# prsinha1/Distributed-Inverse-Problem-Admm

Hardware: AMD Instinct MI355X
Metric: ADMM node-updates/sec (whole node), 512² phantom; rel-Fro vs CPU ref (higher is better)
Workload: dtype f32 samples / f64 state; 1 GPU; C3 (BASELINE.json configs[2] 512^2, 16 graph nodes (ring), 96 angles/node, float32 samples, iso TV, lam=0.02 rho=2, split-Bregman 10x5 CG) on 1 GPU(s), one step = one outer ADMM iteration; image=512, nodes=16, angles_per_node=96, graph=ring, parallelism=graph-node shards x1, batch_streams=1

## Files before the change

### distributed-inverse-problem-admm_amd/admm_hip/_lib.py

```python
from __future__ import annotations

import ctypes as C
import os
import threading

_HERE = os.path.dirname(os.path.abspath(__file__))
LIB_NAME = "libadmm_tomo.so"
LIB_PATH = os.path.join(_HERE, LIB_NAME)

ADMM_DTYPE_F32 = 0
ADMM_DTYPE_F64 = 1
ADMM_TV_ISO = 0
ADMM_TV_ANISO = 1
ADMM_FUSE_MIDPOINT = 0
ADMM_FUSE_WEIGHTED = 1
ADMM_BATCH_KEEP_X = 1
ABI_VERSION = 9
ADMM_MASK_KNN = 0
ADMM_MASK_MST = 1
ADMM_MASK_CHAIN = 2
ADMM_Q_ARITHMETIC = 0
ADMM_Q_HARMONIC = 1
MASK_MAX_NODES = 64
ADMM_FBP_RAMLAK = 0
# ... 52 lines not shown
        ("inc_off", C.c_void_p),
        ("inc_edge", C.c_void_p),
        ("inc_qslot", C.c_void_p),
        ("inc_sign", C.c_void_p),
        ("node_stats", C.c_void_p),
        ("edge_stats", C.c_void_p),
        ("fusion", C.c_int32),
        ("flags", C.c_int32),
        ("y_b", C.c_void_p),
        ("w", C.c_void_p),
        ("x_prev", C.c_void_p),
    ]


SYMBOLS = {
    "admm_abi_version": [],
    "admm_last_error": [],
    "admm_ctx_create": [C.POINTER(C.c_void_p), C.POINTER(Geom), C.c_int, C.c_int, C.c_int],
    "admm_ctx_create_matrix": [C.POINTER(C.c_void_p), C.c_int, C.c_int, C.c_longlong, C.c_void_p, C.c_void_p,
                               C.c_void_p, C.c_int, C.c_int, C.c_int],
    "admm_ctx_destroy": [C.c_void_p],
    "admm_project_fwd": [C.c_void_p, C.c_void_p, C.c_void_p, C.c_int, C.c_void_p],
    "admm_project_adj": [C.c_void_p, C.c_void_p, C.c_void_p, C.c_int, C.c_void_p],
    "admm_column_norms_sq": [C.c_void_p, C.c_void_p, C.c_void_p],
    "admm_tv_grad": [C.c_void_p, C.c_void_p, C.c_void_p, C.c_void_p, C.c_int, C.c_void_p],
    "admm_tv_div": [C.c_void_p, C.c_void_p, C.c_void_p, C.c_void_p, C.c_int, C.c_void_p],
    "admm_batch_bind": [C.c_void_p, C.POINTER(Batch)],
    "admm_batch_atb": [C.c_void_p, C.c_void_p, C.c_void_p],
    "admm_node_update": [C.c_void_p, C.c_void_p],
    "admm_node_update_rounds": [C.c_void_p, C.c_int, C.c_void_p],
    "admm_consensus": [C.c_void_p, C.c_void_p],
    "admm_time_forward": [C.c_void_p, C.c_int, C.c_int, C.c_void_p, C.POINTER(C.c_double)],
    "admm_batch_info": [C.c_void_p, C.POINTER(C.c_int), C.POINTER(C.c_int)],
    "admm_time_back": [C.c_void_p, C.c_void_p, C.POINTER(C.c_double)],
    "admm_consensus_range": [C.c_void_p, C.c_int, C.c_int, C.c_int, C.c_void_p],
    "admm_fwd_plan_info": [C.c_void_p, C.c_int, C.POINTER(C.c_int), C.POINTER(C.c_int),
                           C.POINTER(C.c_double), C.POINTER(C.c_int)],
    "admm_pixel_masks": [C.c_void_p, C.c_int, C.c_int64, C.c_int, C.c_int, C.c_int, C.c_void_p,
                         C.c_void_p, C.c_void_p],
    "admm_chain_orders": [C.POINTER(C.c_uint64), C.c_int, C.c_uint32, C.c_int, C.c_int64, C.c_void_p,
                          C.POINTER(C.c_uint64)],
    "admm_fbp_filter": [C.c_void_p, C.c_void_p, C.c_int, C.c_int, C.c_int, C.c_int, C.c_double, C.c_double,
                        C.c_int, C.c_void_p],
    "admm_image_metrics": [C.c_void_p, C.c_longlong, C.c_void_p, C.c_void_p, C.c_int, C.c_int, C.c_double,
                           C.c_double, C.c_void_p, C.c_void_p, C.c_void_p],
    "admm_image_metrics_work": [C.c_int, C.c_int, C.POINTER(C.c_longlong)],
    "admm_batch_set_ray_weights": [C.c_void_p, C.c_void_p, C.c_void_p],
    "admm_column_norms_sq_weighted": [C.c_void_p, C.c_void_p, C.c_void_p, C.c_void_p],
    "admm_bound_project": [C.c_void_p, C.c_longlong, C.c_void_p, C.c_void_p, C.c_longlong, C.c_void_p, C.c_void_p,
                           C.c_double, C.c_double, C.c_longlong, C.c_int, C.c_void_p, C.c_void_p, C.c_void_p],
    "admm_bound_project_work": [C.c_longlong, C.c_int, C.POINTER(C.c_longlong)],
    "admm_consensus_relaxed": [C.c_void_p, C.c_longlong, C.c_int, C.c_void_p, C.c_void_p, C.c_void_p, C.c_void_p,
                               C.c_void_p, C.c_void_p, C.c_int, C.c_int, C.c_double, C.c_void_p, C.c_void_p,
                               C.c_void_p],
    "admm_consensus_relaxed_work": [C.c_longlong, C.c_int, C.POINTER(C.c_longlong)],
    "admm_bound_project_relaxed": [C.c_void_p, C.c_longlong, C.c_void_p, C.c_void_p, C.c_longlong, C.c_void_p,
                                   C.c_void_p, C.c_double, C.c_double, C.c_longlong, C.c_int, C.c_double, C.c_void_p,
                                   C.c_void_p, C.c_void_p],
    "admm_batch_set_rho": [C.c_void_p, C.c_double, C.c_void_p],
    "admm_node_norms": [C.c_void_p, C.c_longlong, C.c_void_p, C.c_void_p, C.c_void_p, C.c_longlong, C.c_int,
                        C.c_void_p, C.c_void_p, C.c_void_p, C.c_int, C.c_void_p, C.c_void_p, C.c_void_p],
    "admm_node_norms_work": [C.c_longlong, C.c_int, C.POINTER(C.c_longlong)],
    "admm_fuse_absmax": [C.c_void_p, C.c_longlong, C.c_void_p, C.c_longlong, C.c_void_p, C.c_longlong, C.c_int,
                         C.c_int, C.c_void_p, C.c_void_p, C.c_void_p],
    "admm_fuse_absmax_work": [C.c_longlong, C.c_int, C.POINTER(C.c_longlong)],
    "admm_fuse_accumulate": [C.c_void_p, C.c_longlong, C.c_void_p, C.c_longlong, C.c_void_p, C.c_longlong, C.c_int,
# ... 62 lines not shown
```

### distributed-inverse-problem-admm_amd/csrc/admm_tomo.hip

```cpp
#include <hip/hip_runtime.h>

#include <algorithm>
#include <cmath>
#include <cstdio>
#include <cstdlib>
#include <cstring>
#include <initializer_list>
#include <memory>
#include <string>
#include <type_traits>
#include <utility>
#include <vector>

#include "../../include/admm_tomo.h"
#include "fwd_plan.hpp"
#include "kernels.hpp"

using namespace admm;

static_assert(sizeof(FgBlock) == sizeof(int4) && alignof(FgBlock) == alignof(int4), "FgBlock must be an int4");

namespace {
thread_local std::string g_err;

// ... 146 lines not shown
  int wexp = 0;
  static constexpr int kPlans = kFwdPlans;
  FwdPlan plans[kPlans];
  Buf plan_groups_b[kPlans], plan_rng_b[kPlans];
  const FgGroup* plan_groups(int pl) const { return plan_groups_b[pl].as<const FgGroup>(); }
  const FgRange* plan_rng(int pl) const { return plan_rng_b[pl].as<const FgRange>(); }
  int plan_n[kPlans] = {}, plan_blocks[kPlans] = {};
  double plan_staged[kPlans] = {};
  const FgGroup* groups = nullptr;
  const FgRange* rng = nullptr;
  int n_groups = 0;
  bool mirror_half = false;
  Buf fg_order;
  int fg_nblk = 0, fg_order_nch = 0;
  int fg_cpb = 1;
  Stream cap;

  bool csr = false;
  long long nnz = 0;
  Buf f_ptr, f_idx, f_val, t_ptr, t_idx, t_val;

  Buf op_img, op_imgT, op_sino, op_fpart;
  Buf op_order[kPlans];
  int op_nblk[kPlans] = {};
  int op_fpart_key = -1;

  bool bound = false;
  admm_batch b{};
  int vb = 1;
  bool mm = false;
  int bk_staging = 0;
  bool bk_epi_lds = true;
  int n_cu = 0;
  std::unique_ptr<admm_ctx> half;
  Buf xs, xsT, p, pT, Hp, sino, bI, fpart, r, c, d2, e2;
  Buf dsumS;
  Buf wS;
  bool weighted = false;
  Buf x2, p2;
  Buf pring;
  Buf ats;
  std::vector<Event>* tf_ev = nullptr;
  size_t tf_next = 0;
  int tf_kind = 0;
  bool ats_valid = false;
  bool ats_stale = false;
  Buf partH, partS, partD, partE;
  Buf redH;
  int P_back = 0, P_tile = 0, P_fwd = 0, P_edge = 0;
  Graph upd, upd_reuse, cons;

  admm_ctx() = default;
  admm_ctx(const admm_ctx&) = delete;
  admm_ctx& operator=(const admm_ctx&) = delete;
  ~admm_ctx() {
    scope.enter(device);
    (void)hipDeviceSynchronize();
    half.reset();
  }
};

namespace {

int vb_for(int V, int dtype) {
  const int vb = V >= 5 ? 8 : (V >= 3 ? 4 : (V == 2 ? 2 : 1));
  return dtype == ADMM_DTYPE_F64 ? std::min(vb, 4) : vb;
// ... 281 lines not shown
        }
      }
      hipLaunchKernelGGL(kern, grid, dim3(kBkThreads), 0, s, a);
      CHECK_LAUNCH();
      return ADMM_OK;
    }
  }
  back_geom(a, C, C, V);
  const int N = C->g.N;
  constexpr bool kOneImage = MODE == BACK_WSQ || MODE == BACK_WSQW;
  dim3 grid((N + kBTJ - 1) / kBTJ, (N + kBTI - 1) / kBTI, kOneImage ? 1 : (V + VB - 1) / VB);
  if (C->csr) {
    a.csr_ptr = (const int*)C->t_ptr.p;
    a.csr_idx = (const int*)C->t_idx.p;
    a.csr_val = (const T*)C->t_val.p;
    hipLaunchKernelGGL((k_back<T, VB, MODE, true>), grid, dim3(kBkThreads), 0, s, a);
  } else {
    hipLaunchKernelGGL((k_back<T, VB, MODE>), grid, dim3(kBkThreads), 0, s, a);
  }
  CHECK_LAUNCH();
  return ADMM_OK;
}

int back_partitions(admm_ctx* C) {
  const int N = C->g.N;
  const int rows = C->mm ? (N + 1) / 2 : N;
  return ((N + kBTJ - 1) / kBTJ) * ((rows + kBTI - 1) / kBTI);
}
dim3 tile_grid(admm_ctx* C, int nchunks, int vb) {
  const int N = C->g.N, ti = kTile / vb;
  return dim3((N + kTile - 1) / kTile, (N + ti - 1) / ti, nchunks);
}

int launch_reduce(const double* part, int rows, int P, double* out, int G, int ostride, int ooff, hipStream_t s) {
  hipLaunchKernelGGL(k_reduce_rows, dim3(rows), dim3(kBlock), 0, s, part, P, out, G, ostride, ooff);
  CHECK_LAUNCH();
  return ADMM_OK;
}

EdgeIn edge_in(const admm_batch& B) {
  EdgeIn E{};
  E.z = B.z;
  E.y = B.y;
  E.yb = B.fusion == ADMM_FUSE_WEIGHTED ? B.y_b : nullptr;
  E.xp = B.x_prev;
  E.ea = B.edge_a;
  E.eb = B.edge_b;
  return E;
}

template <typename T, int VB>
auto tv_kernel(bool last, bool uin, bool uout) {
  if (last) return uin ? k_tv_update<T, VB, true, true, false> : k_tv_update<T, VB, true, false, false>;
  if (uin) return k_tv_update<T, VB, false, true, true>;
  return uout ? k_tv_update<T, VB, false, false, true> : k_tv_update<T, VB, false, false, false>;
}

template <typename T, int VB>
int enqueue_update(admm_ctx* C, hipStream_t s, bool reuse = false, int rounds = 0) {
  const admm_batch& B = C->b;
  const int V = B.V, N = C->g.N;
  const size_t npix = (size_t)N * N;
  const int nch = (V + VB - 1) / VB;
  T* xs = (T*)C->xs.p;
  T* xsT = (T*)C->xsT.p;
  T* p = (T*)C->p.p;
  T* pT = (T*)C->pT.p;
  T* Hp = (T*)C->Hp.p;
  T* sino = (T*)C->sino.p;
  double* r = (double*)C->r.p;
  double* c = (double*)C->c.p;
  double* redH = (double*)C->redH.p;
  const dim3 tg = tile_grid(C, nch, VB);
  const dim3 cgg((N + kTile - 1) / kTile, (N + kCgRows - 1) / kCgRows, nch);
  const dim3 tvg((N + kTvTile - 1) / kTvTile, (N + EwMap<VB>::TI - 1) / EwMap<VB>::TI, nch);
  const int Pb = C->P_back;

  if (reuse) {
    hipLaunchKernelGGL((k_start_reuse<T, VB>), cgg, dim3(kBlock), 0, s, (const T*)C->ats.p, B.x_ext, edge_in(B),
                       B.q, B.inc_off, B.inc_edge, B.inc_qslot, B.inc_sign, B.atb, c, B.dsum, B.d, B.e, r, p, pT,
                       B.rho, B.mu, N, V);
    CHECK_LAUNCH();
  } else {
  hipLaunchKernelGGL((k_gather<T, VB>), tg, dim3(kBlock), 0, s, B.x_ext, edge_in(B), B.q, B.inc_off, B.inc_edge,
                     B.inc_qslot, B.inc_sign, c, xs, xsT, N, V);
  CHECK_LAUNCH();
  RET((launch_fwd_batch<T, VB, 0>(C, xs, xsT, sino, nullptr, nullptr, V, s)));
  {
    BackArgs<T> a{};
    a.sino = sino;
    a.out_t = p;
    a.out_d = r;
    a.pin = xs;
    a.dsum = B.dsum;
    a.atb = B.atb;
    a.cvec = c;
    a.dvar = B.d;
    a.evar = B.e;
    a.rho = B.rho;
    a.lam = B.lam;
    a.mu = B.mu;
    RET((launch_back<T, VB, BACK_INIT>(C, a, V, s)));
  }
  hipLaunchKernelGGL((k_transpose<T, VB>), tg, dim3(kBlock), 0, s, p, pT, N);
  CHECK_LAUNCH();
  }

  const double tau = B.lam / B.mu;
// ... 27 lines not shown
      a.dsum_s = (const T*)C->dsumS.p;
      a.rho = B.rho;
      a.lam = B.lam;
      a.mu = B.mu;
      Event* bev = nullptr;
      if (C->tf_ev && C->tf_kind == 1 && C->tf_next + 2 <= C->tf_ev->size()) {
        bev = C->tf_ev->data() + C->tf_next;
        C->tf_next += 2;
        HIPCHK(hipEventRecord(bev[0].e, s));
      }
      RET((launch_back<T, VB, BACK_H>(C, a, V, s)));
      if (bev) HIPCHK(hipEventRecord(bev[1].e, s));
      RET(launch_reduce((double*)C->partH.p, 5 * V, Pb, rk, 1, 1, 0, s));
      if (kk + 1 < K) {
        const auto cg = (F == 2) ? k_cg_update<T, VB, false> : k_cg_update<T, VB, true>;
        hipLaunchKernelGGL(cg, cgg, dim3(kBlock), 0, s, xcur, r, pk, pT, Hp, rk, N, V, (F == 2) ? slot[kk + 1] : pk);
        CHECK_LAUNCH();
      }
    }
    const bool last = (t + 1 == Tt);
    PRing<T> pr{};
    pr.K = (F == 2) ? K : 1;
    for (int k = 0; k < pr.K; ++k) pr.p[k] = slot[k];
    T* pout = last ? xs : (F == 2 ? slot[K] : (F == 1 ? slot[1] : slot[0]));
    T* poutT = last ? xsT : pT;
    const bool uin = t > 0 && Tt > 1;
    const bool uout = !last && Tt > 1;
    double* ua = (double*)C->d2.p;
    double* ub = (double*)C->e2.p;
    const double* din = uin ? ((t % 2) ? ua : ub) : dcur;
    const double* ein = ecur;
    double* dout = uout ? ((t % 2) ? ub : ua) : (Tt > 1 ? B.d : dnxt);
    double* eout = uout ? nullptr : (Tt > 1 ? B.e : enxt);
    hipLaunchKernelGGL((tv_kernel<T, VB>(last, uin, uout)), tvg, dim3(kTvThreads), 0, s, xcur, din, ein, dout, eout, r,
                       pout, poutT, tau, B.mu, B.tv_kind, N, V, xnxt, pr, Hp, redH);
    CHECK_LAUNCH();
    if (Tt == 1) {
      std::swap(dcur, dnxt);
      std::swap(ecur, enxt);
    }
    std::swap(xcur, xnxt);
    if (!last) std::swap(slot[0], slot[F == 2 ? K : 1]);
  }
  if (xcur != B.x_ext)
    HIPCHK(hipMemcpyAsync(B.x_ext, xcur, (size_t)V * npix * sizeof(double), hipMemcpyDeviceToDevice, s));
  if (dcur != B.d) {
    HIPCHK(hipMemcpyAsync(B.d, dcur, 2 * V * npix * sizeof(double), hipMemcpyDeviceToDevice, s));
    HIPCHK(hipMemcpyAsync(B.e, ecur, 2 * V * npix * sizeof(double), hipMemcpyDeviceToDevice, s));
  }
  RET((launch_fwd_batch<T, VB, 1>(C, xs, xsT, sino, (const T*)B.b, (double*)C->partS.p, V, s)));
  {
    BackArgs<T> a{};
    a.sino = sino;
    a.part = (double*)C->partD.p;
    a.dsum = B.dsum;
    a.cvec = c;
    a.x = B.x_ext;
    a.phantom = B.phantom;
    a.edges = edge_in(B);
    a.qv = B.q;
    a.inc_off = B.inc_off;
    a.inc_edge = B.inc_edge;
    a.inc_qslot = B.inc_qslot;
    a.inc_sign = B.inc_sign;
    a.rho = B.rho;
    a.lam = B.lam;
    a.mu = B.mu;
    a.tv_kind = B.tv_kind;
// ... 142 lines not shown
  RET(ensure(C->op_sino, vbmax * m * ds));
  RET(ensure(C->op_fpart, (size_t)kFgSeg * vbmax * m * ds));
  for (int v0 = 0; v0 < nimg; v0 += step) {
    const int nc = std::min(step, nimg - v0);
    const T* in = img + (size_t)v0 * npix;
    T* out = sino + (size_t)v0 * m;
    RET(with_vb(vb_for(nc, C->dtype), [&](auto vbc) { return op_forward_chunk<T, decltype(vbc)::value>(C, in, out, nc, s); }));
  }
  return ADMM_OK;
}

}

extern "C" {

int admm_abi_version(void) { return ADMM_ABI_VERSION; }
const char* admm_last_error(void) { return g_err.c_str(); }

int admm_ctx_create(admm_ctx** out, const admm_geom* geom, int dtype, int max_images, int device) {
  if (!out || !geom) return fail(ADMM_E_INVALID, "null argument");
  *out = nullptr;
  const admm_geom g = *geom;
  if (const char* err = check_geom(g, dtype, max_images)) return fail(ADMM_E_INVALID, err);
  GeomTables T;
  if (const char* err = geom_tables(g, dtype, T)) return fail(ADMM_E_INVALID, err);
  FwdPlans P = build_fwd_plans(g, T.fa);
  DEVICE_SCOPE(device);
  std::unique_ptr<admm_ctx> C(new admm_ctx());
  C->g = g;
  C->dtype = dtype;
  C->device = device;
  C->bk_staging = env_word("ADMM_BK_STAGING", {"reg", "dma1", "dma2"});
  C->bk_epi_lds = env_word("ADMM_BK_EPI", {"global"}) == 0;
  HIPCHK(hipDeviceGetAttribute(&C->n_cu, hipDeviceAttributeMultiprocessorCount, device));
  C->max_images = max_images;
  C->npix = g.N * g.N;
  C->mrays = g.n_angles * g.n_det;
  C->Kb = T.Kb;
  C->kbias = T.kbias;
  C->wexp = T.wexp;
  RET(upload(C->fang_b, T.fa));
  RET(upload(C->bang_b, T.ba));
  RET(upload(C->bangc_b, T.bc));
  if (P.fits) {
    for (int pl = 0; pl < admm_ctx::kPlans; ++pl) {
      FwdPlan& Q = P.plan[pl];
      if (Q.groups.empty()) continue;
      RET(upload(C->plan_groups_b[pl], Q.groups));
      RET(upload(C->plan_rng_b[pl], Q.ranges));
      C->plan_n[pl] = (int)Q.groups.size();
      C->plan_blocks[pl] = (int)Q.blocks.size();
      C->plan_staged[pl] = Q.staged;
      C->plans[pl] = std::move(Q);
    }
    select_fwd_plan(C.get(), 0);
  }
  HIPCHK(hipStreamCreateWithFlags(&C->cap.s, hipStreamNonBlocking));
  *out = C.release();
  return ADMM_OK;
}

int admm_ctx_create_matrix(admm_ctx** out, int N, int m, long long nnz, const long long* indptr,
                           const int* indices, const double* values, int dtype, int max_images, int device) {
  if (!out || !indptr || (nnz > 0 && (!indices || !values))) return fail(ADMM_E_INVALID, "null argument");
  *out = nullptr;
  if (N < 2 || N > 4096 || m < 1) return fail(ADMM_E_INVALID, "bad matrix sizes");
// ... 5 lines not shown
    return fail(ADMM_E_INVALID, "batch too large for 32-bit buffer offsets; split it across contexts");
  if (indptr[0] != 0 || indptr[m] != nnz) return fail(ADMM_E_INVALID, "indptr must run from 0 to nnz");
  for (int r = 0; r < m; ++r)
    if (indptr[r + 1] < indptr[r]) return fail(ADMM_E_INVALID, "indptr not non-decreasing");
  for (long long k = 0; k < nnz; ++k)
    if (indices[k] < 0 || (size_t)indices[k] >= npix) return fail(ADMM_E_INVALID, "column index out of range");
  std::vector<int> tptr(npix + 1, 0), tidx((size_t)nnz);
  std::vector<double> tval((size_t)nnz);
  for (long long k = 0; k < nnz; ++k) ++tptr[(size_t)indices[k] + 1];
  for (size_t c = 0; c < npix; ++c) tptr[c + 1] += tptr[c];
  {
    std::vector<int> fill(tptr.begin(), tptr.end() - 1);
    for (int r = 0; r < m; ++r)
      for (long long k = indptr[r]; k < indptr[r + 1]; ++k) {
        const int q = fill[indices[k]]++;
        tidx[q] = r;
        tval[q] = values[k];
      }
  }
  std::vector<int> fptr(m + 1);
  for (int r = 0; r <= m; ++r) fptr[r] = (int)indptr[r];
  DEVICE_SCOPE(device);
  std::unique_ptr<admm_ctx> C(new admm_ctx());
  C->g = admm_geom{};
  C->g.N = N;
  C->g.n_angles = 1;
  C->g.n_det = m;
  C->dtype = dtype;
  C->device = device;
  C->max_images = max_images;
  C->npix = (int)npix;
  C->mrays = m;
  C->csr = true;
  C->nnz = nnz;
  FwdAngle fa{};
  fa.L = 1.0;
  BackAngle ba{};
  BackAngleC bc{};
  auto upv = [&](Buf& b, const std::vector<double>& v) {
    if (dtype == ADMM_DTYPE_F64) return upload(b, v, 16);
    return upload(b, std::vector<float>(v.begin(), v.end()), 16);
  };
  RET(upload(C->f_ptr, fptr, 16));
  RET(upload(C->f_idx, indices, (size_t)nnz * 4, 16));
  RET(upv(C->f_val, std::vector<double>(values, values + nnz)));
  RET(upload(C->t_ptr, tptr, 16));
  RET(upload(C->t_idx, tidx, 16));
  RET(upv(C->t_val, tval));
  RET(upload(C->fang_b, &fa, sizeof(fa)));
  RET(upload(C->bang_b, &ba, sizeof(ba)));
  RET(upload(C->bangc_b, &bc, sizeof(bc)));
  HIPCHK(hipStreamCreateWithFlags(&C->cap.s, hipStreamNonBlocking));
  *out = C.release();
  return ADMM_OK;
}

int admm_ctx_destroy(admm_ctx* C) {
  if (!C) return ADMM_OK;
  delete C;
  return ADMM_OK;
}

int admm_project_fwd(admm_ctx* C, const void* img, void* sino, int nimg, void* stream) {
  if (!C || !img || !sino) return fail(ADMM_E_INVALID, "null argument");
  if (nimg < 1 || nimg > C->max_images) return fail(ADMM_E_INVALID, "nimg out of range");
  hipStream_t s = (hipStream_t)stream;
// ... 401 lines not shown
  return ADMM_OK;
}

int admm_consensus_range(admm_ctx* C, int e0, int e1, int rows, void* stream) {
  if (!C || !C->bound) return fail(ADMM_E_STATE, "no batch bound");
  const admm_batch& B = C->b;
  if (B.z == nullptr || B.fusion != ADMM_FUSE_MIDPOINT)
    return fail(ADMM_E_STATE, "admm_consensus_range needs stored z and midpoint fusion");
  if (e0 < 0 || e1 < e0 || e1 > B.n_edges) return fail(ADMM_E_INVALID, "edge range out of bounds");
  if (rows < 1 || rows > B.n_xext) return fail(ADMM_E_INVALID, "rows out of range");
  DEVICE_SCOPE(C->device);
  return enqueue_consensus_stored(C, e0, e1, (hipStream_t)stream);
}

int admm_time_back(admm_ctx* C, void* stream, double* ms_out) {
  if (!C || !C->bound) return fail(ADMM_E_STATE, "no batch bound");
  if (!ms_out) return fail(ADMM_E_INVALID, "bad argument");
  DEVICE_SCOPE(C->device);
  hipStream_t s = (hipStream_t)stream;
  float ms = 0.f;
  RET(time_in_solve(C, 1, s, &ms));
  *ms_out = (double)ms;
  return ADMM_OK;
}

int admm_batch_info(admm_ctx* C, int* vb, int* mirror) {
  if (!C || !vb || !mirror) return fail(ADMM_E_INVALID, "bad argument");
  if (!C->bound) return fail(ADMM_E_STATE, "no batch bound");
  *vb = C->vb;
  *mirror = C->mm ? 1 : 0;
  return ADMM_OK;
}

int admm_fwd_plan_info(admm_ctx* C, int plan, int* groups, int* blocks, double* staged, int* active) {
  if (!C || plan < 0 || plan >= admm_ctx::kPlans || !groups || !blocks || !staged || !active)
    return fail(ADMM_E_INVALID, "bad argument");
  if (C->mm && C->half) C = C->half.get();
  *groups = C->plan_n[plan];
  *blocks = C->plan_blocks[plan];
  *staged = C->plan_staged[plan];
  *active = (C->plan_n[plan] > 0 && C->groups == C->plan_groups(plan)) ? 1 : 0;
  return ADMM_OK;
}

}
```

### distributed-inverse-problem-admm_amd/csrc/kernels.hpp

```cpp
#pragma once
#include <hip/hip_runtime.h>
#include <stdint.h>

#include <type_traits>

#include "tables.hpp"

namespace admm {

constexpr int kBlock = 256;
constexpr int kTile = 32;
constexpr int kFwdRays = 64;
constexpr int kFwdSegs = 8;
constexpr int kFwdBlock = kFwdRays * kFwdSegs;


__device__ __forceinline__ int clampi(int v, int lo, int hi) { return min(max(v, lo), hi); }

constexpr double kKfBias = 1048576.0;
constexpr unsigned kKfHi = 0x41300000u;
__device__ __forceinline__ void kf_split(double kfb, unsigned& hi, float& fu) {
  const uint64_t b = __builtin_bit_cast(uint64_t, kfb);
  hi = (unsigned)(b >> 32);
  fu = (float)(unsigned)b;
// ... 2195 lines not shown
      }
      tl.t[ii][jj][u] = np[u];
    }
    gstore<T, VB>(pout + sbase + (size_t)pix * VB, np);
  }
  tile_store_T<T, VB, kCgRows, kTile, kBlock>(tl, pT + sbase, N, i0, j0);
}

__device__ __forceinline__ void shrink2(double ux, double uy, double tau, int kind, double& dx, double& dy) {
  if (kind == 0) {
    const double s = sqrt(ux * ux + uy * uy);
    const double f = (s > tau) ? (s - tau) / s : 0.0;
    dx = f * ux;
    dy = f * uy;
  } else {
    dx = copysign(fmax(fabs(ux) - tau, 0.0), ux);
    dy = copysign(fmax(fabs(uy) - tau, 0.0), uy);
  }
}

__device__ __forceinline__ int xcd_remap(int orig, int nwg) {
  const int q = nwg / 8, r = nwg % 8, xcd = orig % 8;
  return (xcd < r ? xcd * (q + 1) : r * (q + 1) + (xcd - r) * q) + orig / 8;
}

constexpr int kMaxCgRing = 8;
template <typename T>
struct PRing {
  const T* p[kMaxCgRing];
  int K;
};
constexpr int kTvTile = 64, kTvThreads = 512;
static_assert(kTvTile == 32 || kTvTile == 64, "TV tile width 32 or 64");
template <typename T, int VB, bool LAST, bool UIN, bool UOUT>
__global__ __launch_bounds__(kTvThreads) void k_tv_update(const double* __restrict__ x, const double* __restrict__ din,
                                                      const double* __restrict__ ein, double* __restrict__ dout,
                                                      double* __restrict__ eout, double* __restrict__ r,
                                                      T* __restrict__ p, T* __restrict__ pT, double tau,
                                                      double mu, int kind, int N, int V, double* __restrict__ xout,
                                                      PRing<T> pr, const T* __restrict__ Hp,
                                                      const double* __restrict__ redH) {
  static_assert(!(LAST && UOUT), "the last round writes d and e");
  using Map = EwMap<VB, kTvTile, kTvThreads>;
  constexpr int TI = Map::TI;
  __shared__ TileT<T, VB, TI, kTvTile> tl;
  const Map mp;
  const int chunk = blockIdx.z, v = chunk * VB + mp.u;
  const bool live = v < V;
  const int npix = N * N;
  const size_t sbase = (size_t)chunk * npix * VB;
  const int wg = xcd_remap(blockIdx.y * gridDim.x + blockIdx.x, gridDim.x * gridDim.y);
  const int i0 = (wg / gridDim.x) * TI, j0 = (wg % gridDim.x) * kTvTile;
  constexpr int PR = TI + 2, PC = kTvTile + 2;
  __shared__ double al_s[kMaxCgRing][VB];
  __shared__ double x_s[VB][PR][PC + 1];
  if ((int)threadIdx.x < VB * pr.K) {
    const int k = threadIdx.x / VB, u = threadIdx.x % VB, vv = chunk * VB + u;
    al_s[k][u] = vv < V ? cg_alpha(redH + (size_t)k * 5 * V + 5 * vv) : 0.0;
  }
  __syncthreads();
  for (int q = threadIdx.x; q < PR * PC; q += kTvThreads) {
    int rr, cc;
    halo_slot<PR, kTvTile>(q, rr, cc);
    const int i = i0 - 1 + rr, j = j0 - 1 + cc;
    if (i < 0 || j < 0 || i >= N || j >= N) continue;
    const int o = i * N + j;
    double xn[VB];
#pragma unroll
    for (int u = 0; u < VB; ++u) {
      const int vq = chunk * VB + u;
      xn[u] = vq < V ? x[(size_t)vq * npix + o] : 0.0;
    }
    T pa[VB], pb[VB];
    gload<T, VB>(pr.p[0] + sbase + (size_t)o * VB, pa);
    for (int k = 0; k < pr.K; ++k) {
      if (k + 1 < pr.K) gload<T, VB>(pr.p[k + 1] + sbase + (size_t)o * VB, pb);
#pragma unroll
      for (int u = 0; u < VB; ++u) xn[u] = fma(al_s[k][u], (double)pa[u], xn[u]);
#pragma unroll
      for (int u = 0; u < VB; ++u) pa[u] = pb[u];
    }
#pragma unroll
    for (int u = 0; u < VB; ++u) x_s[u][rr][cc] = xn[u];
  }
  __syncthreads();
  auto xat = [&](int u, int i, int j) -> double { return x_s[u][i - i0 + 1][j - j0 + 1]; };
  auto gradx = [&](int u, int i, int j, double& gx, double& gy) {
    const double c = xat(u, i, j);
    gx = (i < N - 1) ? xat(u, i + 1, j) - c : 0.0;
    gy = (j < N - 1) ? xat(u, i, j + 1) - c : 0.0;
  };
  const size_t vo = (size_t)(live ? v : 0) * npix;
  const double* ev = ein + 2 * vo;
  if constexpr (!LAST) {
    constexpr int HC = kTvTile + 1, HR = TI + 1;
    __shared__ double qx_s[HR][VB][HC], qy_s[HR][VB][HC];
    for (int q = threadIdx.x; q < HR * HC * VB; q += kTvThreads) {
      int cc, u, rr;
      if (q < HR * VB * kTvTile) {
        cc = 1 + q % kTvTile;
        const int rest = q / kTvTile;
        u = rest % VB;
        rr = rest / VB;
      } else {
        const int h = q - HR * VB * kTvTile;
        cc = 0;
        u = h % VB;
        rr = h / VB;
      }
      const int i = i0 + rr - 1, j = j0 + cc - 1;
      const int vq = chunk * VB + u;
      if (vq >= V || i < 0 || j < 0 || i >= N || j >= N) continue;
      const size_t vqo = (size_t)vq * npix;
      const int o = i * N + j;
      double d0, d1, e0, e1;
      if constexpr (UIN) {
        const double u0 = din[2 * vqo + o], u1 = din[2 * vqo + npix + o];
        shrink2(u0, u1, tau, kind, d0, d1);
        e0 = u0 - d0;
        e1 = u1 - d1;
      } else {
        d0 = din[2 * vqo + o];
        d1 = din[2 * vqo + npix + o];
        e0 = ein[2 * vqo + o];
        e1 = ein[2 * vqo + npix + o];
      }
      double gx, gy, ndx, ndy;
      gradx(u, i, j, gx, gy);
      const double ux = gx + e0, uy = gy + e1;
      shrink2(ux, uy, tau, kind, ndx, ndy);
      const double nex = ux - ndx, ney = uy - ndy;
      qx_s[rr][u][cc] = (ndx - nex) - (d0 - e0);
      qy_s[rr][u][cc] = (ndy - ney) - (d1 - e1);
      if (rr >= 1 && cc >= 1) {
        if constexpr (UOUT) {
          dout[2 * vqo + o] = ux;
          dout[2 * vqo + npix + o] = uy;
        } else {
          dout[2 * vqo + o] = ndx;
          dout[2 * vqo + npix + o] = ndy;
          eout[2 * vqo + o] = nex;
          eout[2 * vqo + npix + o] = ney;
        }
      }
    }
    __syncthreads();
    for (int rw = mp.isub; rw < TI; rw += Map::RPI) {
      const int i = i0 + rw, j = j0 + mp.jj;
      if (i >= N || j >= N) continue;
      const int o = i * N + j;
      T sv = T(0);
      if (live) {
        double kt = 0.0;
        if (i <= N - 2) kt -= qx_s[rw + 1][mp.u][mp.jj + 1];
        if (j <= N - 2) kt -= qy_s[rw + 1][mp.u][mp.jj + 1];
        if (i >= 1) kt += qx_s[rw][mp.u][mp.jj + 1];
        if (j >= 1) kt += qy_s[rw + 1][mp.u][mp.jj];
        double rv = r[vo + o];
        rv = fma(-al_s[pr.K - 1][mp.u], (double)Hp[sbase + (size_t)o * VB + mp.u], rv);
        xout[vo + o] = xat(mp.u, i, j);
        const double rn = fma(mu, kt, rv);
        r[vo + o] = rn;
        sv = (T)rn;
      }
      p[sbase + (size_t)o * VB + mp.u] = sv;
      tl.t[rw][mp.jj][mp.u] = sv;
    }
  } else {
    for (int rw = mp.isub; rw < TI; rw += Map::RPI) {
      const int i = i0 + rw, j = j0 + mp.jj;
      if (i >= N || j >= N) continue;
      const int o = i * N + j;
      T sv = T(0);
      if (live) {
        double e0, e1, gx, gy, ndx, ndy;
        if constexpr (UIN) {
          const double u0 = din[2 * vo + o], u1 = din[2 * vo + npix + o];
          double d0, d1;
          shrink2(u0, u1, tau, kind, d0, d1);
          e0 = u0 - d0;
          e1 = u1 - d1;
        } else {
          e0 = ev[o];
          e1 = ev[npix + o];
        }
        gradx(mp.u, i, j, gx, gy);
        const double ux = gx + e0, uy = gy + e1;
        shrink2(ux, uy, tau, kind, ndx, ndy);
        const double nex = ux - ndx, ney = uy - ndy;
        dout[2 * vo + o] = ndx;
        dout[2 * vo + npix + o] = ndy;
        eout[2 * vo + o] = nex;
        eout[2 * vo + npix + o] = ney;
        const double xn = xat(mp.u, i, j);
        xout[vo + o] = xn;
        sv = (T)xn;
      }
      p[sbase + (size_t)o * VB + mp.u] = sv;
      tl.t[rw][mp.jj][mp.u] = sv;
    }
  }
  tile_store_T<T, VB, TI, kTvTile, kTvThreads>(tl, pT + sbase, N, i0, j0);
}

template <typename T, int VB>
__global__ void k_pack_d(const double* __restrict__ in, T* __restrict__ out, int L, int V, double scale) {
  const int q = blockIdx.x * blockDim.x + threadIdx.x;
  const int chunk = blockIdx.y, v0 = chunk * VB;
  if (q >= L) return;
  const T sc = (T)scale;
  T s[VB];
#pragma unroll
  for (int u = 0; u < VB; ++u) s[u] = (v0 + u < V) ? (T)in[(size_t)(v0 + u) * L + q] * sc : T(0);
  gstore<T, VB>(out + ((size_t)chunk * L + q) * VB, s);
}

template <typename T, int VB>
__global__ void k_pack(const T* __restrict__ in, T* __restrict__ out, int L, int V) {
  const int q = blockIdx.x * blockDim.x + threadIdx.x;
  const int chunk = blockIdx.y, v0 = chunk * VB;
  if (q >= L) return;
  T s[VB];
#pragma unroll
  for (int u = 0; u < VB; ++u) s[u] = (v0 + u < V) ? in[(size_t)(v0 + u) * L + q] : T(0);
  gstore<T, VB>(out + ((size_t)chunk * L + q) * VB, s);
}

template <typename T, int VB>
__global__ void k_pack_w(const T* __restrict__ in, const T* __restrict__ wts, T* __restrict__ out, int L, int V) {
  const int q = blockIdx.x * blockDim.x + threadIdx.x;
  const int chunk = blockIdx.y, v0 = chunk * VB;
  if (q >= L) return;
  T s[VB], w[VB];
  gload<T, VB>(wts + ((size_t)chunk * L + q) * VB, w);
#pragma unroll
// ... 200 lines not shown
```

### include/admm_tomo.h

```cpp
#ifndef ADMM_TOMO_H
#define ADMM_TOMO_H

#include <stdint.h>

#ifdef __cplusplus
extern "C" {
#endif

#define ADMM_ABI_VERSION 9

#define ADMM_OK 0
#define ADMM_E_INVALID (-1)
#define ADMM_E_HIP (-2)
#define ADMM_E_STATE (-3)

#define ADMM_DTYPE_F32 0
#define ADMM_DTYPE_F64 1

#define ADMM_TV_ISO 0
#define ADMM_TV_ANISO 1

#define ADMM_FUSE_MIDPOINT 0
#define ADMM_FUSE_WEIGHTED 1

// ... 60 lines not shown

    double* x_prev;
} admm_batch;

int admm_abi_version(void);
const char* admm_last_error(void);

int admm_ctx_create(admm_ctx** out, const admm_geom* geom, int dtype, int max_images, int device);
int admm_ctx_create_matrix(admm_ctx** out, int N, int m, long long nnz, const long long* indptr,
                           const int* indices, const double* values, int dtype, int max_images, int device);
int admm_ctx_destroy(admm_ctx* ctx);


int admm_project_fwd(admm_ctx* ctx, const void* img, void* sino, int nimg, void* stream);
int admm_project_adj(admm_ctx* ctx, const void* sino, void* img, int nimg, void* stream);
int admm_column_norms_sq(admm_ctx* ctx, double* W, void* stream);
int admm_column_norms_sq_weighted(admm_ctx* ctx, const void* w, double* W, void* stream);
int admm_tv_grad(admm_ctx* ctx, const double* x, double* gx, double* gy, int nimg, void* stream);
int admm_tv_div(admm_ctx* ctx, const double* px, const double* py, double* out, int nimg,
                void* stream);


int admm_batch_bind(admm_ctx* ctx, const admm_batch* batch);
int admm_batch_atb(admm_ctx* ctx, double* atb_out, void* stream);
int admm_batch_set_ray_weights(admm_ctx* ctx, const void* w, void* stream);
int admm_batch_update_ray_weights(admm_ctx* ctx, const void* w, void* stream);
int admm_batch_refresh_kept(admm_ctx* ctx, void* stream);
int admm_node_update(admm_ctx* ctx, void* stream);
int admm_node_update_rounds(admm_ctx* ctx, int tv_iters, void* stream);
int admm_consensus(admm_ctx* ctx, void* stream);
int admm_time_forward(admm_ctx* ctx, int reps, int in_solve, void* stream, double* ms_out);
int admm_fwd_plan_info(admm_ctx* ctx, int plan, int* groups, int* blocks, double* staged, int* active);
int admm_batch_info(admm_ctx* ctx, int* vb, int* mirror);
int admm_consensus_range(admm_ctx* ctx, int e0, int e1, int rows, void* stream);
int admm_time_back(admm_ctx* ctx, void* stream, double* ms_out);


#define ADMM_MASK_KNN 0
#define ADMM_MASK_MST 1
#define ADMM_MASK_CHAIN 2
#define ADMM_Q_ARITHMETIC 0
#define ADMM_Q_HARMONIC 1
#define ADMM_MASK_MAX_NODES 64

int admm_pixel_masks(const double* W, int V, int64_t n, int strategy, int k, int q_mode,
                     const int32_t* orders, uint8_t* keep, void* stream);
int admm_chain_orders(const uint64_t pcg[4], int has_uint32, uint32_t uinteger, int V, int64_t n,
                      int32_t* orders, uint64_t pcg_out[6]);


#define ADMM_FBP_RAMLAK 0
#define ADMM_FBP_SHEPP_LOGAN 1
#define ADMM_FBP_HANN 2

int admm_fbp_filter(const void* sino, void* out, int dtype, int n_angles, int n_det, int nimg,
                    double det_spacing, double scale, int filter, void* stream);


int admm_image_metrics(const double* img, long long img_stride, const double* ref, const uint8_t* mask,
                       int N, int nimg, double c1, double c2, double* work, double* out, void* stream);
int admm_image_metrics_work(int N, int nimg, long long* n_doubles);


int admm_bound_project(const double* x, long long x_stride, double* w, double* f, long long wf_stride,
                       const double* lo_map, const double* hi_map, double lo, double hi, long long n,
                       int nimg, double* work, double* out, void* stream);
// ... 42 lines not shown
```

Baseline: 2261 node-updates/s.

## Sweep TV kernel over multiple row tiles per workgroup, carrying halo rows

The TV update kernel now processes up to four consecutive row tiles per workgroup. It carries the overlapping x halo rows and q boundary row in LDS between tiles instead of recomputing them, which avoids re-reading the p-ring and x data for halos and re-evaluating shrink on boundary rows. Sweep depth is picked by default (4 for non-last rounds, 1 for the last) and halved until the grid still has at least twice as many workgroups as CUs. In exchange, the q buffers move into a struct that is empty for the last round, the grid shrinks, and each workgroup runs serially over more tiles.

```diff
diff --git a/distributed-inverse-problem-admm_amd/admm_hip/_lib.py b/distributed-inverse-problem-admm_amd/admm_hip/_lib.py
--- a/distributed-inverse-problem-admm_amd/admm_hip/_lib.py
+++ b/distributed-inverse-problem-admm_amd/admm_hip/_lib.py
@@ -108,6 +108,8 @@
     "admm_consensus": [C.c_void_p, C.c_void_p],
     "admm_time_forward": [C.c_void_p, C.c_int, C.c_int, C.c_void_p, C.POINTER(C.c_double)],
     "admm_batch_info": [C.c_void_p, C.POINTER(C.c_int), C.POINTER(C.c_int)],
+    "admm_tv_sweep_plan": [C.c_int, C.c_int, C.c_int, C.c_int, C.c_int, C.c_int, C.POINTER(C.c_int),
+                           C.POINTER(C.c_int)],
     "admm_time_back": [C.c_void_p, C.c_void_p, C.POINTER(C.c_double)],
     "admm_consensus_range": [C.c_void_p, C.c_int, C.c_int, C.c_int, C.c_void_p],
     "admm_fwd_plan_info": [C.c_void_p, C.c_int, C.POINTER(C.c_int), C.POINTER(C.c_int),
diff --git a/distributed-inverse-problem-admm_amd/csrc/admm_tomo.hip b/distributed-inverse-problem-admm_amd/csrc/admm_tomo.hip
--- a/distributed-inverse-problem-admm_amd/csrc/admm_tomo.hip
+++ b/distributed-inverse-problem-admm_amd/csrc/admm_tomo.hip
@@ -202,6 +202,7 @@
   int bk_staging = 0;
   bool bk_epi_lds = true;
   int n_cu = 0;
+  int tv_sweep = 0;
   std::unique_ptr<admm_ctx> half;
   Buf xs, xsT, p, pT, Hp, sino, bI, fpart, r, c, d2, e2;
   Buf dsumS;
@@ -549,6 +550,16 @@
   return dim3((N + kTile - 1) / kTile, (N + ti - 1) / ti, nchunks);
 }
 
+constexpr int kTvSweeps[] = {0, 1, 2, 4};
+int tv_sweep_depth(int N, int vb, int nchunks, int n_cu, int forced, bool last, dim3* grid) {
+  const long gx = (N + kTvTile - 1) / kTvTile, ty = (N + kTile / vb - 1) / (kTile / vb);
+  int R = forced ? forced : (last ? 1 : 4);
+  if (!forced)
+    while (R > 1 && gx * ((ty + R - 1) / R) * nchunks < 2L * n_cu) R /= 2;
+  *grid = dim3(gx, (ty + R - 1) / R, nchunks);
+  return R;
+}
+
 int launch_reduce(const double* part, int rows, int P, double* out, int G, int ostride, int ooff, hipStream_t s) {
   hipLaunchKernelGGL(k_reduce_rows, dim3(rows), dim3(kBlock), 0, s, part, P, out, G, ostride, ooff);
   CHECK_LAUNCH();
@@ -590,7 +601,6 @@
   double* redH = (double*)C->redH.p;
   const dim3 tg = tile_grid(C, nch, VB);
   const dim3 cgg((N + kTile - 1) / kTile, (N + kCgRows - 1) / kCgRows, nch);
-  const dim3 tvg((N + kTvTile - 1) / kTvTile, (N + EwMap<VB>::TI - 1) / EwMap<VB>::TI, nch);
   const int Pb = C->P_back;
 
   if (reuse) {
@@ -684,8 +694,10 @@
     const double* ein = ecur;
     double* dout = uout ? ((t % 2) ? ub : ua) : (Tt > 1 ? B.d : dnxt);
     double* eout = uout ? nullptr : (Tt > 1 ? B.e : enxt);
+    dim3 tvg;
+    const int tvs = tv_sweep_depth(N, VB, nch, C->n_cu, C->tv_sweep, last, &tvg);
     hipLaunchKernelGGL((tv_kernel<T, VB>(last, uin, uout)), tvg, dim3(kTvThreads), 0, s, xcur, din, ein, dout, eout, r,
-                       pout, poutT, tau, B.mu, B.tv_kind, N, V, xnxt, pr, Hp, redH);
+                       pout, poutT, tau, B.mu, B.tv_kind, N, V, xnxt, pr, Hp, redH, tvs);
     CHECK_LAUNCH();
     if (Tt == 1) {
       std::swap(dcur, dnxt);
@@ -894,6 +906,7 @@
   C->device = device;
   C->bk_staging = env_word("ADMM_BK_STAGING", {"reg", "dma1", "dma2"});
   C->bk_epi_lds = env_word("ADMM_BK_EPI", {"global"}) == 0;
+  C->tv_sweep = kTvSweeps[env_word("ADMM_TV_SWEEP", {"1", "2", "4"})];
   HIPCHK(hipDeviceGetAttribute(&C->n_cu, hipDeviceAttributeMultiprocessorCount, device));
   C->max_images = max_images;
   C->npix = g.N * g.N;
@@ -965,6 +978,8 @@
   C->npix = (int)npix;
   C->mrays = m;
   C->csr = true;
+  C->tv_sweep = kTvSweeps[env_word("ADMM_TV_SWEEP", {"1", "2", "4"})];
+  HIPCHK(hipDeviceGetAttribute(&C->n_cu, hipDeviceAttributeMultiprocessorCount, device));
   C->nnz = nnz;
   FwdAngle fa{};
   fa.L = 1.0;
@@ -1432,6 +1447,18 @@
   return ADMM_OK;
 }
 
+int admm_tv_sweep_plan(int N, int vb, int nchunks, int n_cu, int forced, int last, int* depth, int* grid) {
+  if (N < 1 || (vb != 1 && vb != 2 && vb != 4 && vb != 8) || nchunks < 1 || n_cu < 1 ||
+      (forced != 0 && forced != 1 && forced != 2 && forced != 4) || !depth || !grid)
+    return fail(ADMM_E_INVALID, "bad argument");
+  dim3 g;
+  *depth = tv_sweep_depth(N, vb, nchunks, n_cu, forced, last != 0, &g);
+  grid[0] = (int)g.x;
+  grid[1] = (int)g.y;
+  grid[2] = (int)g.z;
+  return ADMM_OK;
+}
+
 int admm_fwd_plan_info(admm_ctx* C, int plan, int* groups, int* blocks, double* staged, int* active) {
   if (!C || plan < 0 || plan >= admm_ctx::kPlans || !groups || !blocks || !staged || !active)
     return fail(ADMM_E_INVALID, "bad argument");
diff --git a/distributed-inverse-problem-admm_amd/csrc/kernels.hpp b/distributed-inverse-problem-admm_amd/csrc/kernels.hpp
--- a/distributed-inverse-problem-admm_amd/csrc/kernels.hpp
+++ b/distributed-inverse-problem-admm_amd/csrc/kernels.hpp
@@ -2251,6 +2251,12 @@
 };
 constexpr int kTvTile = 64, kTvThreads = 512;
 static_assert(kTvTile == 32 || kTvTile == 64, "TV tile width 32 or 64");
+template <int VB, int ROWS, int COLS>
+struct TvQ {
+  double x[ROWS][VB][COLS], y[ROWS][VB][COLS];
+};
+template <int VB, int COLS>
+struct TvQ<VB, 0, COLS> {};
 template <typename T, int VB, bool LAST, bool UIN, bool UOUT>
 __global__ __launch_bounds__(kTvThreads) void k_tv_update(const double* __restrict__ x, const double* __restrict__ din,
                                                       const double* __restrict__ ein, double* __restrict__ dout,
@@ -2258,7 +2264,7 @@
                                                       T* __restrict__ p, T* __restrict__ pT, double tau,
                                                       double mu, int kind, int N, int V, double* __restrict__ xout,
                                                       PRing<T> pr, const T* __restrict__ Hp,
-                                                      const double* __restrict__ redH) {
+                                                      const double* __restrict__ redH, int sweep) {
   static_assert(!(LAST && UOUT), "the last round writes d and e");
   using Map = EwMap<VB, kTvTile, kTvThreads>;
   constexpr int TI = Map::TI;
@@ -2269,157 +2275,183 @@
   const int npix = N * N;
   const size_t sbase = (size_t)chunk * npix * VB;
   const int wg = xcd_remap(blockIdx.y * gridDim.x + blockIdx.x, gridDim.x * gridDim.y);
-  const int i0 = (wg / gridDim.x) * TI, j0 = (wg % gridDim.x) * kTvTile;
+  const int j0 = (wg % gridDim.x) * kTvTile;
   constexpr int PR = TI + 2, PC = kTvTile + 2;
+  constexpr int HC = kTvTile + 1, HR = TI + 1;
   __shared__ double al_s[kMaxCgRing][VB];
   __shared__ double x_s[VB][PR][PC + 1];
+  __shared__ TvQ<VB, LAST ? 0 : HR, HC> qs;
   if ((int)threadIdx.x < VB * pr.K) {
     const int k = threadIdx.x / VB, u = threadIdx.x % VB, vv = chunk * VB + u;
     al_s[k][u] = vv < V ? cg_alpha(redH + (size_t)k * 5 * V + 5 * vv) : 0.0;
   }
   __syncthreads();
-  for (int q = threadIdx.x; q < PR * PC; q += kTvThreads) {
-    int rr, cc;
-    halo_slot<PR, kTvTile>(q, rr, cc);
-    const int i = i0 - 1 + rr, j = j0 - 1 + cc;
-    if (i < 0 || j < 0 || i >= N || j >= N) continue;
-    const int o = i * N + j;
-    double xn[VB];
-#pragma unroll
-    for (int u = 0; u < VB; ++u) {
-      const int vq = chunk * VB + u;
-      xn[u] = vq < V ? x[(size_t)vq * npix + o] : 0.0;
-    }
-    T pa[VB], pb[VB];
-    gload<T, VB>(pr.p[0] + sbase + (size_t)o * VB, pa);
-    for (int k = 0; k < pr.K; ++k) {
-      if (k + 1 < pr.K) gload<T, VB>(pr.p[k + 1] + sbase + (size_t)o * VB, pb);
-#pragma unroll
-      for (int u = 0; u < VB; ++u) xn[u] = fma(al_s[k][u], (double)pa[u], xn[u]);
-#pragma unroll
-      for (int u = 0; u < VB; ++u) pa[u] = pb[u];
-    }
-#pragma unroll
-    for (int u = 0; u < VB; ++u) x_s[u][rr][cc] = xn[u];
-  }
-  __syncthreads();
-  auto xat = [&](int u, int i, int j) -> double { return x_s[u][i - i0 + 1][j - j0 + 1]; };
-  auto gradx = [&](int u, int i, int j, double& gx, double& gy) {
-    const double c = xat(u, i, j);
-    gx = (i < N - 1) ? xat(u, i + 1, j) - c : 0.0;
-    gy = (j < N - 1) ? xat(u, i, j + 1) - c : 0.0;
-  };
   const size_t vo = (size_t)(live ? v : 0) * npix;
   const double* ev = ein + 2 * vo;
-  if constexpr (!LAST) {
-    constexpr int HC = kTvTile + 1, HR = TI + 1;
-    __shared__ double qx_s[HR][VB][HC], qy_s[HR][VB][HC];
-    for (int q = threadIdx.x; q < HR * HC * VB; q += kTvThreads) {
-      int cc, u, rr;
-      if (q < HR * VB * kTvTile) {
-        cc = 1 + q % kTvTile;
-        const int rest = q / kTvTile;
-        u = rest % VB;
-        rr = rest / VB;
-      } else {
-        const int h = q - HR * VB * kTvTile;
-        cc = 0;
-        u = h % VB;
-        rr = h / VB;
-      }
-      const int i = i0 + rr - 1, j = j0 + cc - 1;
-      const int vq = chunk * VB + u;
-      if (vq >= V || i < 0 || j < 0 || i >= N || j >= N) continue;
-      const size_t vqo = (size_t)vq * npix;
+  auto tile = [&](auto carried, const int i0) {
+    constexpr bool CARRIED = decltype(carried)::value;
+    constexpr int XR0 = CARRIED ? 2 : 0, QR0 = CARRIED ? 1 : 0;
+    for (int q = threadIdx.x; q < (PR - XR0) * PC; q += kTvThreads) {
+      int rr, cc;
+      halo_slot<PR - XR0, kTvTile>(q, rr, cc);
+      rr += XR0;
+      const int i = i0 - 1 + rr, j = j0 - 1 + cc;
+      if (i < 0 || j < 0 || i >= N || j >= N) continue;
       const int o = i * N + j;
-      double d0, d1, e0, e1;
-      if constexpr (UIN) {
-        const double u0 = din[2 * vqo + o], u1 = din[2 * vqo + npix + o];
-        shrink2(u0, u1, tau, kind, d0, d1);
-        e0 = u0 - d0;
-        e1 = u1 - d1;
-      } else {
-        d0 = din[2 * vqo + o];
-        d1 = din[2 * vqo + npix + o];
-        e0 = ein[2 * vqo + o];
-        e1 = ein[2 * vqo + npix + o];
-      }
-      double gx, gy, ndx, ndy;
-      gradx(u, i, j, gx, gy);
-      const double ux = gx + e0, uy = gy + e1;
-      shrink2(ux, uy, tau, kind, ndx, ndy);
-      const double nex = ux - ndx, ney = uy - ndy;
-      qx_s[rr][u][cc] = (ndx - nex) - (d0 - e0);
-      qy_s[rr][u][cc] = (ndy - ney) - (d1 - e1);
-      if (rr >= 1 && cc >= 1) {
-        if constexpr (UOUT) {
-          dout[2 * vqo + o] = ux;
-          dout[2 * vqo + npix + o] = uy;
+      double xn[VB];
+#pragma unroll
+      for (int u = 0; u < VB; ++u) {
+        const int vq = chunk * VB + u;
+        xn[u] = vq < V ? x[(size_t)vq * npix + o] : 0.0;
+      }
+      T pa[VB], pb[VB];
+      gload<T, VB>(pr.p[0] + sbase + (size_t)o * VB, pa);
+      for (int k = 0; k < pr.K; ++k) {
+        if (k + 1 < pr.K) gload<T, VB>(pr.p[k + 1] + sbase + (size_t)o * VB, pb);
+#pragma unroll
+        for (int u = 0; u < VB; ++u) xn[u] = fma(al_s[k][u], (double)pa[u], xn[u]);
+#pragma unroll
+        for (int u = 0; u < VB; ++u) pa[u] = pb[u];
+      }
+#pragma unroll
+      for (int u = 0; u < VB; ++u) x_s[u][rr][cc] = xn[u];
+    }
+    __syncthreads();
+    auto xat = [&](int u, int i, int j) -> double { return x_s[u][i - i0 + 1][j - j0 + 1]; };
+    auto gradx = [&](int u, int i, int j, double& gx, double& gy) {
+      const double c = xat(u, i, j);
+      gx = (i < N - 1) ? xat(u, i + 1, j) - c : 0.0;
+      gy = (j < N - 1) ? xat(u, i, j + 1) - c : 0.0;
+    };
+    if constexpr (!LAST) {
+      auto& qx_s = qs.x;
+      auto& qy_s = qs.y;
+      constexpr int QR = HR - QR0;
+      for (int q = threadIdx.x; q < QR * HC * VB; q += kTvThreads) {
+        int cc, u, rr;
+        if (q < QR * VB * kTvTile) {
+          cc = 1 + q % kTvTile;
+          const int rest = q / kTvTile;
+          u = rest % VB;
+          rr = QR0 + rest / VB;
         } else {
-          dout[2 * vqo + o] = ndx;
-          dout[2 * vqo + npix + o] = ndy;
-          eout[2 * vqo + o] = nex;
-          eout[2 * vqo + npix + o] = ney;
+          const int h = q - QR * VB * kTvTile;
+          cc = 0;
+          u = h % VB;
+          rr = QR0 + h / VB;
         }
-      }
-    }
-    __syncthreads();
-    for (int rw = mp.isub; rw < TI; rw += Map::RPI) {
-      const int i = i0 + rw, j = j0 + mp.jj;
-      if (i >= N || j >= N) continue;
-      const int o = i * N + j;
-      T sv = T(0);
-      if (live) {
-        double kt = 0.0;
-        if (i <= N - 2) kt -= qx_s[rw + 1][mp.u][mp.jj + 1];
-        if (j <= N - 2) kt -= qy_s[rw + 1][mp.u][mp.jj + 1];
-        if (i >= 1) kt += qx_s[rw][mp.u][mp.jj + 1];
-        if (j >= 1) kt += qy_s[rw + 1][mp.u][mp.jj];
-        double rv = r[vo + o];
-        rv = fma(-al_s[pr.K - 1][mp.u], (double)Hp[sbase + (size_t)o * VB + mp.u], rv);
-        xout[vo + o] = xat(mp.u, i, j);
-        const double rn = fma(mu, kt, rv);
-        r[vo + o] = rn;
-        sv = (T)rn;
-      }
-      p[sbase + (size_t)o * VB + mp.u] = sv;
-      tl.t[rw][mp.jj][mp.u] = sv;
-    }
-  } else {
-    for (int rw = mp.isub; rw < TI; rw += Map::RPI) {
-      const int i = i0 + rw, j = j0 + mp.jj;
-      if (i >= N || j >= N) continue;
-      const int o = i * N + j;
-      T sv = T(0);
-      if (live) {
-        double e0, e1, gx, gy, ndx, ndy;
+        const int i = i0 + rr - 1, j = j0 + cc - 1;
+        const int vq = chunk * VB + u;
+        if (vq >= V || i < 0 || j < 0 || i >= N || j >= N) continue;
+        const size_t vqo = (size_t)vq * npix;
+        const int o = i * N + j;
+        double d0, d1, e0, e1;
         if constexpr (UIN) {
-          const double u0 = din[2 * vo + o], u1 = din[2 * vo + npix + o];
-          double d0, d1;
+          const double u0 = din[2 * vqo + o], u1 = din[2 * vqo + npix + o];
           shrink2(u0, u1, tau, kind, d0, d1);
           e0 = u0 - d0;
           e1 = u1 - d1;
         } else {
-          e0 = ev[o];
-          e1 = ev[npix + o];
+          d0 = din[2 * vqo + o];
+          d1 = din[2 * vqo + npix + o];
+          e0 = ein[2 * vqo + o];
+          e1 = ein[2 * vqo + npix + o];
         }
-        gradx(mp.u, i, j, gx, gy);
+        double gx, gy, ndx, ndy;
+        gradx(u, i, j, gx, gy);
         const double ux = gx + e0, uy = gy + e1;
         shrink2(ux, uy, tau, kind, ndx, ndy);
         const double nex = ux - ndx, ney = uy - ndy;
-        dout[2 * vo + o] = ndx;
-        dout[2 * vo + npix + o] = ndy;
-        eout[2 * vo + o] = nex;
-        eout[2 * vo + npix + o] = ney;
-        const double xn = xat(mp.u, i, j);
-        xout[vo + o] = xn;
-        sv = (T)xn;
-      }
-      p[sbase + (size_t)o * VB + mp.u] = sv;
-      tl.t[rw][mp.jj][mp.u] = sv;
-    }
-  }
-  tile_store_T<T, VB, TI, kTvTile, kTvThreads>(tl, pT + sbase, N, i0, j0);
+        qx_s[rr][u][cc] = (ndx - nex) - (d0 - e0);
+        qy_s[rr][u][cc] = (ndy - ney) - (d1 - e1);
+        if (rr >= 1 && cc >= 1) {
+          if constexpr (UOUT) {
+            dout[2 * vqo + o] = ux;
+            dout[2 * vqo + npix + o] = uy;
+          } else {
+            dout[2 * vqo + o] = ndx;
+            dout[2 * vqo + npix + o] = ndy;
+            eout[2 * vqo + o] = nex;
+            eout[2 * vqo + npix + o] = ney;
+          }
+        }
+      }
+      __syncthreads();
+      for (int rw = mp.isub; rw < TI; rw += Map::RPI) {
+        const int i = i0 + rw, j = j0 + mp.jj;
+        if (i >= N || j >= N) continue;
+        const int o = i * N + j;
+        T sv = T(0);
+        if (live) {
+          double kt = 0.0;
+          if (i <= N - 2) kt -= qx_s[rw + 1][mp.u][mp.jj + 1];
+          if (j <= N - 2) kt -= qy_s[rw + 1][mp.u][mp.jj + 1];
+          if (i >= 1) kt += qx_s[rw][mp.u][mp.jj + 1];
+          if (j >= 1) kt += qy_s[rw + 1][mp.u][mp.jj];
+          double rv = r[vo + o];
+          rv = fma(-al_s[pr.K - 1][mp.u], (double)Hp[sbase + (size_t)o * VB + mp.u], rv);
+          xout[vo + o] = xat(mp.u, i, j);
+          const double rn = fma(mu, kt, rv);
+          r[vo + o] = rn;
+          sv = (T)rn;
+        }
+        p[sbase + (size_t)o * VB + mp.u] = sv;
+        tl.t[rw][mp.jj][mp.u] = sv;
+      }
+    } else {
+      for (int rw = mp.isub; rw < TI; rw += Map::RPI) {
+        const int i = i0 + rw, j = j0 + mp.jj;
+        if (i >= N || j >= N) continue;
+        const int o = i * N + j;
+        T sv = T(0);
+        if (live) {
+          double e0, e1, gx, gy, ndx, ndy;
+          if constexpr (UIN) {
+            const double u0 = din[2 * vo + o], u1 = din[2 * vo + npix + o];
+            double d0, d1;
+            shrink2(u0, u1, tau, kind, d0, d1);
+            e0 = u0 - d0;
+            e1 = u1 - d1;
+          } else {
+            e0 = ev[o];
+            e1 = ev[npix + o];
+          }
+          gradx(mp.u, i, j, gx, gy);
+          const double ux = gx + e0, uy = gy + e1;
+          shrink2(ux, uy, tau, kind, ndx, ndy);
+          const double nex = ux - ndx, ney = uy - ndy;
+          dout[2 * vo + o] = ndx;
+          dout[2 * vo + npix + o] = ndy;
+          eout[2 * vo + o] = nex;
+          eout[2 * vo + npix + o] = ney;
+          const double xn = xat(mp.u, i, j);
+          xout[vo + o] = xn;
+          sv = (T)xn;
+        }
+        p[sbase + (size_t)o * VB + mp.u] = sv;
+        tl.t[rw][mp.jj][mp.u] = sv;
+      }
+    }
+    tile_store_T<T, VB, TI, kTvTile, kTvThreads>(tl, pT + sbase, N, i0, j0);
+  };
+  const int ib = (wg / gridDim.x) * TI * sweep;
+  tile(std::false_type{}, ib);
+  for (int t = 1; t < sweep; ++t) {
+    const int i0 = ib + t * TI;
+    if (i0 >= N) break;
+    for (int q = threadIdx.x; q < VB * 2 * PC; q += kTvThreads) {
+      const int u = q / (2 * PC), rr = (q / PC) % 2, cc = q % PC;
+      x_s[u][rr][cc] = x_s[u][TI + rr][cc];
+    }
+    if constexpr (!LAST)
+      for (int q = threadIdx.x; q < VB * HC; q += kTvThreads) {
+        const int u = q / HC, cc = q % HC;
+        qs.x[0][u][cc] = qs.x[TI][u][cc];
+        qs.y[0][u][cc] = qs.y[TI][u][cc];
+      }
+    __syncthreads();
+    tile(std::true_type{}, i0);
+  }
 }
 
 template <typename T, int VB>
diff --git a/include/admm_tomo.h b/include/admm_tomo.h
--- a/include/admm_tomo.h
+++ b/include/admm_tomo.h
@@ -116,6 +116,7 @@
 int admm_time_forward(admm_ctx* ctx, int reps, int in_solve, void* stream, double* ms_out);
 int admm_fwd_plan_info(admm_ctx* ctx, int plan, int* groups, int* blocks, double* staged, int* active);
 int admm_batch_info(admm_ctx* ctx, int* vb, int* mirror);
+int admm_tv_sweep_plan(int N, int vb, int nchunks, int n_cu, int forced, int last, int* depth, int* grid);
 int admm_consensus_range(admm_ctx* ctx, int e0, int e1, int rows, void* stream);
 int admm_time_back(admm_ctx* ctx, void* stream, double* ms_out);
 
```

Measured after the change: 2264 node-updates/s, median of 6. No clear change (+0.1%).
